# jmloveyj/ros_navigation

Measured on AMD Instinct MI355X. Metric: replan cycles/sec (HIMM+VFH++A*) on 4096x4096 grid, higher is better.
Workload: dtype int32; 1 GPU; full replan loop on 4096x4096 f32 grid (res 0.05 m); one step = one turn of the 20-stage A* pipeline = 20 passes of [100032-ray HIMM batch + fused compose -> 256 VFH+ poses -> 256 grid-A* queries (one launch)]; 30% rectangle obstacles (seed 2); 4 ray batches / pose sets / query sets in rotation; cycles_per_pass=256, rays_per_pass=100032, rotating_input_sets=4, astar_queries_checked=15360, astar_queries_answered=15360, astar_bucket_width=128000, astar_pipeline_depth=20, parallelism=query-sharded x1, full=False

## Files before the change

### ros_navigation_amd/csrc/astar.hip

```cpp
#include "engine.hpp"

#include <algorithm>
#include <cfloat>
#include <cmath>
#include <cstdlib>
#include <cstring>
#include <chrono>
#include <thread>
#include <vector>

using namespace rna;

namespace {

constexpr int COST_D = 1414;

struct HostTrace {
  bool on = getenv("RNA_HOST_TRACE") != nullptr;
  double us[8] = {};
  long n = 0, queries = 0;
  std::chrono::steady_clock::time_point t;
  void start() { if (on) t = std::chrono::steady_clock::now(); }
  void lap(int k) {
    if (!on) return;
// ... 65 lines not shown
          for (int c = skip; c < e->cu_count && c < 512; ++c) mask[c >> 5] |= 1u << (c & 31);
          RNA_HIP(e, hipExtStreamCreateWithCUMask(&a.side[d], (uint32_t)words, mask));
        } else {
          RNA_HIP(e, hipStreamCreateWithPriority(&a.side[d], hipStreamNonBlocking, prio_lo));
        }
      }
      RNA_HIP(e, hipEventCreateWithFlags(&a.done[d], hipEventDisableTiming));
      RNA_HIP(e, hipEventCreateWithFlags(&a.snap_done[d], hipEventDisableTiming));
    }
    a.snap_pending[d] = false;
    a.busy[d] = false;
    a.stage_seq[d] = 0;
  }
  if (a.depth > 1) {
    RNA_HIP(e, hipEventCreateWithFlags(&a.ev_init, hipEventDisableTiming));
    RNA_HIP(e, hipEventCreateWithFlags(&a.ev_prep, hipEventDisableTiming));
    a.ring_n = 2 * a.depth;
    a.ring_stride = tsa_ring_bytes(e, a.max_queries);
    if ((rc = dev_alloc(e, &a.ring_mem, a.ring_stride * (size_t)a.ring_n)) != RNA_OK) return rc;
    RNA_HIP(e, hipMemsetAsync(a.ring_mem, 0, a.ring_stride * (size_t)a.ring_n, e->stream));
    for (int r = 0; r < a.ring_n; ++r) {
      RNA_HIP(e, hipEventCreateWithFlags(&a.ring_free[r], hipEventDisableTiming));
      a.ring_used[r] = false;
    }
  }
  if (a.g_retry[0]) {
    RNA_HIP(e, hipHostMalloc(reinterpret_cast<void**>(&a.retry_flag), AstarDevice::MAX_DEPTH * sizeof(int), hipHostMallocCoherent));
    for (int d = 0; d < AstarDevice::MAX_DEPTH; ++d) a.retry_flag[d] = 0;
  }
  a.launches = 0;
  if ((rc = dev_alloc(e, &a.queries_dev, (size_t)a.max_queries)) != RNA_OK) { astar_release(e); return rc; }
  if ((rc = dev_alloc(e, &a.results_dev, (size_t)a.max_queries)) != RNA_OK) { astar_release(e); return rc; }
  return RNA_OK;
}

static int alloc_stages(rna_engine* e) {
  const int rc = alloc_stages_impl(e);
  if (rc != RNA_OK) {
    const std::string why = e->err;
    (void)astar_release(e);
    e->err = why;
  }
  return rc;
}
// ... 171 lines not shown
#ifdef RNA_TSA_STATS
  tsa_stats_dump();
#endif
  for (int d = 0; d < AstarDevice::MAX_DEPTH; ++d) {
    dev_free(&a.g[d]); dev_free(&a.rev[d]);
    if (a.tsa_aux[d]) { (void)hipFree(a.tsa_aux[d]); a.tsa_aux[d] = nullptr; }
    dev_free(&a.g_retry[d]);
    if (a.tsa_aux_retry[d]) { (void)hipFree(a.tsa_aux_retry[d]); a.tsa_aux_retry[d] = nullptr; }
    if (a.side[d]) { (void)hipStreamDestroy(a.side[d]); a.side[d] = nullptr; }
    if (a.done[d]) { (void)hipEventDestroy(a.done[d]); a.done[d] = nullptr; }
    if (a.snap_done[d]) { (void)hipEventDestroy(a.snap_done[d]); a.snap_done[d] = nullptr; }
    a.snap_pending[d] = false;
    a.busy[d] = false;
  }
  if (a.ev_init) { (void)hipEventDestroy(a.ev_init); a.ev_init = nullptr; }
  if (a.ev_prep) { (void)hipEventDestroy(a.ev_prep); a.ev_prep = nullptr; }
  for (int r = 0; r < AstarDevice::MAX_RING; ++r) {
    if (a.ring_free[r]) { (void)hipEventDestroy(a.ring_free[r]); a.ring_free[r] = nullptr; }
    a.ring_used[r] = false;
  }
  dev_free(&a.ring_mem);
  a.ring_n = 0;
  if (a.retry_flag) { (void)hipHostFree(a.retry_flag); a.retry_flag = nullptr; }
  for (int d = 0; d < AstarDevice::MAX_DEPTH; ++d) a.retry_armed[d] = false;
  dev_free(&a.queries_dev); dev_free(&a.results_dev); dev_free(&a.paths_dev);
  a.paths_cap = 0;
  a.last_queries = nullptr; a.last_results = nullptr; a.last_n = 0;
  return RNA_OK;
}
}

extern "C" int rna_astar_configure(rna_engine* e, int max_queries, int queue_capacity, int bucket_width) {
  if (!e || max_queries < 0 || queue_capacity < 0 || bucket_width < 0) return RNA_EINVAL;
  if (bucket_width != 0 && bucket_width < 2 * COST_D) return fail(e, RNA_EINVAL, "bucket_width must be >= 2828");
  RNA_ENTER(e);
  RNA_HIP(e, hipStreamSynchronize(e->stream));
  AstarDevice& a = e->astar;
// ... 145 lines not shown
```

### ros_navigation_amd/csrc/astar_tile.hip

```cpp
#include "engine.hpp"
#include <algorithm>
#include <cstring>
#include <vector>

using namespace rna;

namespace rna {

constexpr int TI = 64, TJ = 16;
constexpr int TILE_WORDS = TI * TJ;
constexpr int AUX_WORDS = 64;
constexpr int MASK_STRIDE = TILE_WORDS + 32 + 128;
constexpr int TSA_WAVES = 8;
constexpr int TSA_WAVES_PER_EU = 8;
constexpr int TSA_HPASS = 4;
constexpr int TSA_IDLE_SLEEP = 4;
constexpr int TSA_PRIO_FIRST = 0;
constexpr int TSA_BT_PRIO = 3;
constexpr int TSA_SCOPE = __HIP_MEMORY_SCOPE_AGENT;
constexpr int TSA_MAX_TILE_WORDS = 2048;
constexpr int COST_S = 1000, COST_D = 1414;
constexpr int INF = 0x7fffffff;
constexpr int KU = 0x40000000;
constexpr int SCR_CNT = 84 + 192 + 48 + 64;
// ... 78 lines not shown
  unsigned* paux;
  unsigned* tmap;
  unsigned* owner;
  int* nalloc;
  uint8_t* nbr_tm;
  int* perm;
  int* ticket;
  int cap;
};
__host__ __device__ inline size_t tsa_align256(size_t x) { return (x + 255) & ~(size_t)255; }
constexpr int TSA_COUNTER_WORDS = 16;
__host__ __device__ inline unsigned long long* tsa_counters_of(const TsaStage& S) {
  return reinterpret_cast<unsigned long long*>(reinterpret_cast<char*>(S.nalloc) - TSA_COUNTER_WORDS * sizeof(unsigned long long));
}

__global__ void __launch_bounds__(256) tsa_snapshot_kernel(const uint8_t* __restrict__ nbr, int rows, int cols, int tiles_i, int tiles_j,
                                                             uint8_t* __restrict__ nbr_tm, int s0, int s1) {
  __shared__ unsigned s_free[256];
  const int a = threadIdx.x & 63, bq = threadIdx.x >> 6;
  for (int t = blockIdx.x; t < tiles_i * tiles_j; t += gridDim.x) {
    const int i = (t % tiles_i) * TI + a, j0 = (t / tiles_i) * TJ + bq * 4;
    unsigned v = 0u;
    if (i < rows) {
      const int bi = i + s0 >= rows ? i + s0 - rows : i + s0;
#pragma unroll
      for (int k = 0; k < 4; ++k)
        if (j0 + k < cols) {
          const int bj = j0 + k + s1 >= cols ? j0 + k + s1 - cols : j0 + k + s1;
          v |= (unsigned)nbr[(size_t)bj * rows + bi] << (8 * k);
        }
    }
    uint8_t* out = nbr_tm + (size_t)t * MASK_STRIDE;
    reinterpret_cast<unsigned*>(out)[a * 4 + bq] = v;
    if (a == 0) reinterpret_cast<unsigned*>(out + TILE_WORDS)[bq] = v;
    if (a == TI - 1) reinterpret_cast<unsigned*>(out + TILE_WORDS + 16)[bq] = v;
    s_free[threadIdx.x] = (((v & 0xffu) != 0u) ? 1u : 0u) | (((v & 0xff00u) != 0u) ? 2u : 0u) | (((v & 0xff0000u) != 0u) ? 4u : 0u) |
                          (((v & 0xff000000u) != 0u) ? 8u : 0u);
    __syncthreads();
    if (bq == 0)
      reinterpret_cast<unsigned short*>(out + TILE_WORDS + 32)[a] =
          (unsigned short)(s_free[a] | (s_free[64 + a] << 4) | (s_free[128 + a] << 8) | (s_free[192 + a] << 12));
    __syncthreads();
  }
}
__global__ void __launch_bounds__(256) tsa_prepare_kernel(TsaStage S, const rna_astar_query* __restrict__ queries, int n, int rows, int cols,
                                                          int ranked, int* __restrict__ served) {
  extern __shared__ int s_key[];
  if (threadIdx.x == 0) *S.ticket = 0;
  if (served && threadIdx.x < TSA_RETRY) served[threadIdx.x] = -1;
  if (served && threadIdx.x == TSA_RETRY) served[TSA_RETRY] = 0;
  if (!ranked) {
    for (int i = threadIdx.x; i < n; i += blockDim.x) S.perm[i] = i;
    return;
  }
  const int ncell = rows * cols;
  for (int i = threadIdx.x; i < n; i += blockDim.x) {
    const rna_astar_query q = queries[i];
    int key = -1;
    if (q.start >= 0 && q.goal >= 0 && q.start < ncell && q.goal < ncell) {
      const int di = abs(q.start % rows - q.goal % rows), dj = abs(q.start / rows - q.goal / rows);
      key = di > dj ? di : dj;
    }
    s_key[i] = key;
  }
  __syncthreads();
  for (int i = threadIdx.x; i < n; i += blockDim.x) {
    const int ki = s_key[i];
    int rank = 0;
    for (int j = 0; j < n; ++j) {
      const int kj = s_key[j];
      rank += (kj > ki || (kj == ki && j < i)) ? 1 : 0;
    }
    S.perm[rank] = i;
  }
}
__global__ void tsa_fill_pages_kernel(uint4* __restrict__ p, size_t n4) {
  const size_t step = (size_t)gridDim.x * blockDim.x;
  for (size_t w = (size_t)blockIdx.x * blockDim.x + threadIdx.x; w < n4; w += step) p[w] = make_uint4(0u, 0u, 0u, 0u);
}

#ifdef RNA_TSA_STATS
__device__ unsigned long long g_tsa_stat[32];
#define TSA_T(var) const unsigned long long var = wall_clock64()
#define TSA_ACC(slot, t0, t1) tsa_acc[slot] += (unsigned long long)((t1) - (t0))
#define TSA_CNT(slot, v) tsa_acc[slot] += (unsigned long long)(v)
#define TSA_ACC_PARAM , unsigned long long* tsa_acc
#define TSA_ACC_ARG , tsa_acc
#else
// ... 1240 lines not shown
  return RNA_OK;
}
int tsa_stage_prepare(rna_engine* e, int slot) {
  const TsaStage S = tsa_stage_view(e, slot);
  const size_t pages = (size_t)e->astar.max_queries * ((size_t)S.cap + 1);
  hipLaunchKernelGGL(tsa_fill_pages_kernel, dim3(8192), dim3(256), 0, e->stream, reinterpret_cast<uint4*>(S.pages),
                     pages * (TILE_WORDS + AUX_WORDS) / 4);
  RNA_HIP(e, hipGetLastError());
  return RNA_OK;
}

size_t tsa_ring_bytes(const rna_engine* e, int max_queries) {
  return 256 + tsa_align256((size_t)max_queries * sizeof(int)) + tsa_align256((size_t)tsa_ntile(e) * MASK_STRIDE);
}
static_assert(sizeof(TsaLaunch) <= sizeof(AstarDevice::last_launch[0]), "AstarDevice::last_launch holds a TsaLaunch");

int tsa_retry_launch(rna_engine* e, int slot, hipStream_t search_stream, int count) {
  AstarDevice& a = e->astar;
  TsaLaunch A;
  memcpy(&A, a.last_launch[slot], sizeof(A));
  A.retry = 1;
  A.retry_count = nullptr;
  A.S2 = tsa_retry_view(e, slot, A.S);
  for (int base = 0; base < count; base += TSA_RETRY) {
    A.retry_base = base;
    const int wgs = std::min(TSA_RETRY, count - base);
    if (a.depth > 1) hipLaunchKernelGGL((tsa_search_kernel<TSA_WAVES, true>), dim3(wgs), dim3(TSA_WAVES * 64), a.last_lds[slot], search_stream, A);
    else hipLaunchKernelGGL((tsa_search_kernel<16, true>), dim3(wgs), dim3(16 * 64), a.last_lds[slot], search_stream, A);
    RNA_HIP(e, hipGetLastError());
  }
// ... 8 lines not shown
  TsaStage S = tsa_stage_view(e, slot);
  hipStream_t prep_stream = search_stream;
  int ring = -1;
  if (ev_init) {
    ring = (int)(a.launches % (unsigned long long)a.ring_n);
    char* base = a.ring_mem + (size_t)ring * a.ring_stride;
    S.ticket = reinterpret_cast<int*>(base);
    S.perm = reinterpret_cast<int*>(base + 256);
    S.nbr_tm = reinterpret_cast<uint8_t*>(base + 256 + tsa_align256((size_t)a.max_queries * sizeof(int)));
    { const int rc = side_stream(e, &prep_stream); if (rc != RNA_OK) return rc; }
    RNA_HIP(e, hipEventRecord(ev_init, init_stream));
    RNA_HIP(e, hipStreamWaitEvent(prep_stream, ev_init, 0));
    if (a.ring_used[ring]) RNA_HIP(e, hipStreamWaitEvent(prep_stream, a.ring_free[ring], 0));
  }
  {
    KernelTimer kt(e, RNA_K_ASTAR_INIT, prep_stream);
    hipLaunchKernelGGL(tsa_snapshot_kernel, dim3(std::min(ti * tj, 4096)), dim3(256), 0, prep_stream, e->nbr, rows, cols, ti, tj, S.nbr_tm,
                       e->geom.start[0], e->geom.start[1]);
    RNA_HIP(e, hipGetLastError());
  }
  if (ev_init) {
    RNA_HIP(e, hipEventRecord(a.snap_done[slot], prep_stream));
    a.snap_pending[slot] = true;
  }
  {
    KernelTimer kt(e, RNA_K_ASTAR_RESET, prep_stream);
    const int ranked = n <= 2048 ? 1 : 0;
    hipLaunchKernelGGL(tsa_prepare_kernel, dim3(1), dim3(256), ranked ? (size_t)n * sizeof(int) : 0, prep_stream, S, q_dev, n, rows, cols, ranked,
                       a.g_retry[slot] ? tsa_retry_served(e, slot) : nullptr);
    RNA_HIP(e, hipGetLastError());
  }
  if (ev_init) {
    RNA_HIP(e, hipEventRecord(a.ev_prep, prep_stream));
    RNA_HIP(e, hipStreamWaitEvent(search_stream, a.ev_prep, 0));
  }
  {
    KernelTimer kt(e, RNA_K_ASTAR_SEARCH, search_stream);
    const size_t nt_bytes = (size_t)((ti * tj + 31) / 32) * sizeof(unsigned);
    TsaLaunch A;
    memset(&A, 0, sizeof(A));
    A.rows = rows; A.cols = cols; A.tiles_i = ti; A.tiles_j = tj; A.s0 = e->geom.start[0]; A.s1 = e->geom.start[1];
    A.queries = q_dev; A.S = S; A.bucket_width = a.bucket_width; A.paths = paths_dev; A.max_path_len = max_len;
    A.rev_all = a.rev[slot]; A.rev_cap = a.rev_cap; A.results = res_dev;
    A.retry = 0; A.n = n; A.S2 = S;
    A.prio_first = a.depth > 1 ? TSA_PRIO_FIRST : 0;
    if (const char* pf = getenv("RNA_TSA_PRIO_FIRST")) A.prio_first = atoi(pf);
    size_t lds_dyn = 4 * nt_bytes;
    if (const char* pad = getenv("RNA_TSA_LDS_PAD")) lds_dyn += (size_t)atoi(pad);
    const bool can_retry = a.g_retry[slot] != nullptr && a.retry_flag != nullptr;
// ... 83 lines not shown
```

### ros_navigation_amd/csrc/compose_dev.hpp

```cpp
#pragma once
#include "engine.hpp"

namespace rna {

__device__ __forceinline__ bool cell_blocked(float v) { return !(v != v) && v > 0.0f; }

constexpr int COMPOSE_BLK_BYTES = (TILE + 2) * (TILE + 2);

__device__ __forceinline__ void compose_nbr_tile(uint8_t* __restrict__ blk, int tt, uint8_t* __restrict__ nbr, float* __restrict__ master,
                                                 const float* __restrict__ laser, const unsigned* __restrict__ dirty,
                                                 unsigned* __restrict__ next_dirty, int rows, int cols, int tiles_i, int tiles_j) {
  const int ti = tt % tiles_i, tj = tt / tiles_i;
  const unsigned char* dflag = reinterpret_cast<const unsigned char*>(dirty);
  unsigned dmask = 0u;
  for (int dj = -1; dj <= 1; ++dj)
    for (int di = -1; di <= 1; ++di) {
      const int a = ti + di, b = tj + dj;
      if (a < 0 || b < 0 || a >= tiles_i || b >= tiles_j) continue;
      if (dflag[b * tiles_i + a]) dmask |= 1u << ((dj + 1) * 3 + di + 1);
    }
  if (threadIdx.x == 0) reinterpret_cast<volatile unsigned char*>(next_dirty)[tj * tiles_i + ti] = 0;
  if (!dmask) return;
  const bool own = (dmask >> 4) & 1u;
  __syncthreads();
  const int i0 = ti * TILE - 1, j0 = tj * TILE - 1;
  for (int k = threadIdx.x; k < (TILE + 2) * (TILE + 2); k += blockDim.x) {
// ... 17 lines not shown
    if (i >= rows || j >= cols) continue;
    const uint8_t* c = &blk[(lj + 1) * (TILE + 2) + (li + 1)];
    constexpr int S = TILE + 2;
    unsigned m = 0;
    if (!c[0]) {
      const bool up = !c[-1], dn = !c[1], lf = !c[-S], rt = !c[S];
      if (lf && up && !c[-S - 1]) m |= 1u;
      if (lf) m |= 2u;
      if (lf && dn && !c[-S + 1]) m |= 4u;
      if (up) m |= 8u;
      if (dn) m |= 16u;
      if (rt && up && !c[S - 1]) m |= 32u;
      if (rt) m |= 64u;
      if (rt && dn && !c[S + 1]) m |= 128u;
    }
    nbr[(size_t)j * rows + i] = (uint8_t)m;
  }
}

}
```

### ros_navigation_amd/csrc/engine.hip

```cpp
#include "engine.hpp"
#include "compose_dev.hpp"

#include <cmath>
#include <dirent.h>
#include <unistd.h>
#include <cstdlib>
#include <cstring>
#include <limits>

using namespace rna;

__global__ void fill_f32_kernel(float* __restrict__ p, size_t n, float v) {
  size_t i = (size_t)blockIdx.x * blockDim.x + threadIdx.x;
  const size_t stride = (size_t)gridDim.x * blockDim.x;
  for (; i < n; i += stride) p[i] = v;
}

__global__ void compose_dirty_tiles_kernel(float* __restrict__ master, const float* __restrict__ laser,
                                           const unsigned* __restrict__ dirty, int rows, int cols, int tiles_i) {
  const int ti = blockIdx.x, tj = blockIdx.y;
  const int t = tj * tiles_i + ti;
  if (!reinterpret_cast<const unsigned char*>(dirty)[t]) return;
  const int i0 = ti * TILE, j0 = tj * TILE;
  const int li = threadIdx.x & (TILE - 1);
  for (int c = threadIdx.x >> 6; c < TILE; c += 4) {
    const int i = i0 + li, j = j0 + c;
    if (i < rows && j < cols) {
      const size_t lin = (size_t)j * rows + i;
      master[lin] = laser[lin];
    }
  }
}


__global__ void nbr_mask_tiles_kernel(uint8_t* __restrict__ nbr, const float* __restrict__ master,
                                      const unsigned* __restrict__ dirty, int all, int rows, int cols,
                                      int tiles_i, int tiles_j, int s0, int s1) {
  const int ti = blockIdx.x, tj = blockIdx.y;
  if (!all) {
    bool need = false;
    for (int dj = -1; dj <= 1 && !need; ++dj)
      for (int di = -1; di <= 1; ++di) {
        const int a = ti + di, b = tj + dj;
        if (a < 0 || b < 0 || a >= tiles_i || b >= tiles_j) continue;
        const int t = b * tiles_i + a;
        if (reinterpret_cast<const unsigned char*>(dirty)[t]) { need = true; break; }
      }
    if (!need) return;
  }
  __shared__ uint8_t blk[(TILE + 2) * (TILE + 2)];
  const int i0 = ti * TILE - 1, j0 = tj * TILE - 1;
  for (int k = threadIdx.x; k < (TILE + 2) * (TILE + 2); k += blockDim.x) {
// ... 18 lines not shown
    unsigned m = 0;
    if (!c[0]) {
      const bool up = !c[-1], dn = !c[1], lf = !c[-S], rt = !c[S];
      if (lf && up && !c[-S - 1]) m |= 1u;
      if (lf) m |= 2u;
      if (lf && dn && !c[-S + 1]) m |= 4u;
      if (up) m |= 8u;
      if (dn) m |= 16u;
      if (rt && up && !c[S - 1]) m |= 32u;
      if (rt) m |= 64u;
      if (rt && dn && !c[S + 1]) m |= 128u;
    }
    int bi = i + s0, bj = j + s1;
    if (bi >= rows) bi -= rows;
    if (bj >= cols) bj -= cols;
    nbr[(size_t)bj * rows + bi] = (uint8_t)m;
  }
}

__global__ void __launch_bounds__(256) compose_nbr_tiles_kernel(uint8_t* __restrict__ nbr, float* __restrict__ master, const float* __restrict__ laser,
                                                                const unsigned* __restrict__ dirty, unsigned* __restrict__ next_dirty, int rows,
                                                                int cols, int tiles_i, int tiles_j) {
  __shared__ uint8_t blk[(TILE + 2) * (TILE + 2)];
  for (int tt = blockIdx.x; tt < tiles_i * tiles_j; tt += gridDim.x)
    compose_nbr_tile(blk, tt, nbr, master, laser, dirty, next_dirty, rows, cols, tiles_i, tiles_j);
}

__global__ void clear_region_kernel(float* __restrict__ p, int rows, int i0, int ni, int j0, int nj) {
  const size_t n = (size_t)ni * nj;
  size_t k = (size_t)blockIdx.x * blockDim.x + threadIdx.x;
  const size_t stride = (size_t)gridDim.x * blockDim.x;
  const float nanv = __int_as_float(0x7fc00000);
  for (; k < n; k += stride) {
    const int i = i0 + (int)(k % ni), j = j0 + (int)(k / ni);
    p[(size_t)j * rows + i] = nanv;
  }
}

__global__ void __launch_bounds__(256) pack_tiles_kernel(const float* __restrict__ layer, int rows, int tiles_i,
                                                         const int32_t* __restrict__ tiles, int wi0, int wi1, int wj0,
// ... 115 lines not shown
      const int words = (prop.multiProcessorCount + 31) / 32 < 16 ? (prop.multiProcessorCount + 31) / 32 : 16;
      if (hipExtStreamCreateWithCUMask(&e->stream, (uint32_t)words, mask) != hipSuccess) return bail(RNA_EHIP);
    } else if (hipStreamCreateWithPriority(&e->stream, hipStreamNonBlocking, prio_hi) != hipSuccess) return bail(RNA_EHIP);
  }
  for (int l = 0; l < RNA_NUM_LAYERS; ++l) {
    if ((rc = dev_alloc(e, &e->layer[l], e->ncell)) != RNA_OK) return bail(rc);
    if ((rc = fill_layer(e, e->layer[l], std::numeric_limits<float>::quiet_NaN())) != RNA_OK) return bail(rc);
  }
  const size_t words = ((size_t)e->tiles_i * e->tiles_j + 3) / 4;
  if ((rc = dev_alloc(e, &e->dirty_tiles, words)) != RNA_OK) return bail(rc);
  if (hipMemsetAsync(e->dirty_tiles, 0, words * sizeof(unsigned), e->stream) != hipSuccess) return bail(RNA_EHIP);
  if ((rc = dev_alloc(e, &e->last_dirty, words)) != RNA_OK) return bail(rc);
  if (hipMemsetAsync(e->last_dirty, 0, words * sizeof(unsigned), e->stream) != hipSuccess) return bail(RNA_EHIP);
  if ((rc = dev_alloc(e, &e->nbr, e->ncell)) != RNA_OK) return bail(rc);
  e->nbr_all_dirty = true;
  if (hipStreamSynchronize(e->stream) != hipSuccess) return bail(RNA_EHIP);
  *out = e;
  return RNA_OK;
}

extern "C" void rna_destroy(rna_engine* e) {
  if (!e) return;
  (void)hipSetDevice(e->device);
  if (e->stream) (void)sync_all(e);
  himm_release(e);
  vfh_release(e);
  astar_release(e);
  footprint_release(e);
  goal_field_release(e);
  for (int l = 0; l < RNA_NUM_LAYERS; ++l) dev_free(&e->layer[l]);
  dev_free(&e->dirty_tiles);
  dev_free(&e->last_dirty);
  dev_free(&e->tile_list);
  dev_free(&e->nbr);
  (void)profile_flush(e);
  for (hipEvent_t ev : e->free_events) (void)hipEventDestroy(ev);
  e->free_events.clear();
  if (e->vfh_stream) (void)hipStreamDestroy(e->vfh_stream);
  if (e->ev_vfh_go) (void)hipEventDestroy(e->ev_vfh_go);
  if (e->ev_vfh_done) (void)hipEventDestroy(e->ev_vfh_done);
  if (e->stream) (void)hipStreamDestroy(e->stream);
  delete e;
}

extern "C" int rna_get_geometry(const rna_engine* e, rna_geometry* o) {
  if (!e || !o) return RNA_EINVAL;
  for (int a = 0; a < 2; ++a) {
    o->length[a] = e->geom.len[a];
    o->position[a] = e->geom.pos[a];
// ... 417 lines not shown
  int src = sync_all(e);
  if (src != RNA_OK) return src;
  for (auto& slot : e->prof) {
    for (auto& pr : slot.pending) {
      float ms = 0;
      if (hipEventElapsedTime(&ms, pr.first, pr.second) == hipSuccess) { slot.total_ms += ms; slot.launches += 1; }
      e->free_events.push_back(pr.first);
      e->free_events.push_back(pr.second);
    }
    slot.pending.clear();
  }
  e->pending_events = 0;
  return RNA_OK;
}

int map_prepare_nbr(rna_engine* e) {
  if (!e->nbr_all_dirty) return RNA_OK;
  { const int rc = side_join(e); if (rc != RNA_OK) return rc; }
  if (e->robot_r > 0.0) {
    const int rc = footprint_refresh(e, 1);
    if (rc != RNA_OK) return rc;
    e->nbr_all_dirty = false;
    return RNA_OK;
  }
  KernelTimer kt(e, RNA_K_NBRMASK);
  hipLaunchKernelGGL(nbr_mask_tiles_kernel, dim3(e->tiles_i, e->tiles_j), dim3(256), 0, e->stream, e->nbr,
                     e->layer[RNA_LAYER_MASTER], e->dirty_tiles, 1, e->geom.size[0], e->geom.size[1], e->tiles_i,
                     e->tiles_j, e->geom.start[0], e->geom.start[1]);
  RNA_HIP(e, hipGetLastError());
  e->nbr_all_dirty = false;
  return RNA_OK;
}

}

extern "C" int rna_compose_master(rna_engine* e, int mode) {
  if (!e || (mode != 0 && mode != 1)) return RNA_EINVAL;
  RNA_ENTER(e);
  e->map_epoch++;
  const size_t words = ((size_t)e->tiles_i * e->tiles_j + 3) / 4;
  const bool full = (mode == 1) || e->laser_all_dirty || e->master_diverged;
  const bool moved = e->geom.start[0] != 0 || e->geom.start[1] != 0;
  if (!full && !moved && !e->nbr_all_dirty && e->robot_r == 0.0) {
    KernelTimer kt(e, RNA_K_COMPOSE);
    static const int wgs_per_cu = [] { const char* v = getenv("RNA_COMPOSE_WGS_PER_CU"); const int n = v ? atoi(v) : 0; return n > 0 ? n : 16; }();
    hipLaunchKernelGGL(compose_nbr_tiles_kernel, dim3(std::min(e->tiles_i * e->tiles_j, wgs_per_cu * e->cu_count)), dim3(256), 0, e->stream, e->nbr,
                       e->layer[RNA_LAYER_MASTER], e->layer[RNA_LAYER_LASER], e->dirty_tiles, e->last_dirty, e->geom.size[0],
                       e->geom.size[1], e->tiles_i, e->tiles_j);
    RNA_HIP(e, hipGetLastError());
    std::swap(e->dirty_tiles, e->last_dirty);
    return RNA_OK;
  }
  {
    KernelTimer kt(e, RNA_K_COMPOSE);
    if (full) {
      RNA_HIP(e, hipMemcpyAsync(e->layer[RNA_LAYER_MASTER], e->layer[RNA_LAYER_LASER], e->ncell * sizeof(float),
                                hipMemcpyDeviceToDevice, e->stream));
    } else {
      hipLaunchKernelGGL(compose_dirty_tiles_kernel, dim3(e->tiles_i, e->tiles_j), dim3(256), 0, e->stream,
                         e->layer[RNA_LAYER_MASTER], e->layer[RNA_LAYER_LASER], e->dirty_tiles, e->geom.size[0],
                         e->geom.size[1], e->tiles_i);
      RNA_HIP(e, hipGetLastError());
    }
  }
  if (e->laser_all_dirty || e->master_diverged || moved) {
    e->nbr_all_dirty = true;
  } else if (!e->nbr_all_dirty && e->robot_r > 0.0) {
    const int rc = footprint_refresh(e, 0);
    if (rc != RNA_OK) return rc;
  } else if (!e->nbr_all_dirty) {
    KernelTimer kt(e, RNA_K_NBRMASK);
    hipLaunchKernelGGL(nbr_mask_tiles_kernel, dim3(e->tiles_i, e->tiles_j), dim3(256), 0, e->stream, e->nbr,
                       e->layer[RNA_LAYER_MASTER], e->dirty_tiles, 0, e->geom.size[0], e->geom.size[1], e->tiles_i,
                       e->tiles_j, 0, 0);
    RNA_HIP(e, hipGetLastError());
  }
  if (full) {
    RNA_HIP(e, hipMemsetAsync(e->last_dirty, 1, words * sizeof(unsigned), e->stream));
  } else {
    RNA_HIP(e, hipMemcpyAsync(e->last_dirty, e->dirty_tiles, words * sizeof(unsigned), hipMemcpyDeviceToDevice, e->stream));
  }
  RNA_HIP(e, hipMemsetAsync(e->dirty_tiles, 0, words * sizeof(unsigned), e->stream));
  e->laser_all_dirty = false;
  e->master_diverged = false;
  return RNA_OK;
}

extern "C" int rna_move(rna_engine* e, double nx, double ny, int* moved) {
  if (!e) return RNA_EINVAL;
// ... 78 lines not shown
```

### ros_navigation_amd/csrc/engine.hpp

```cpp
#pragma once

#include <hip/hip_runtime.h>

#include <cstdint>
#include <cstdio>
#include <string>
#include <vector>

#include "../../include/rna.h"
#include "gridmath.hpp"

namespace rna {

constexpr int TILE = 64;

struct HimmSlot { int cell; int head; int len; int offset; };

struct HimmScratch {
  int cap_rays = 0;
  int n_slots = 0;
  rna_ray* rays_dev = nullptr;
  int4* desc = nullptr;
  int* ncells = nullptr;
  int* next = nullptr;
  HimmSlot* slots = nullptr;
  int* seqs = nullptr;
  unsigned* before = nullptr;
  unsigned* after = nullptr;
  int* total = nullptr;
// ... 45 lines not shown
  int32_t* g_retry[MAX_DEPTH] = {};
  void* tsa_aux_retry[MAX_DEPTH] = {};
  hipStream_t side[MAX_DEPTH] = {};
  hipEvent_t done[MAX_DEPTH] = {};
  hipEvent_t snap_done[MAX_DEPTH] = {};
  bool snap_pending[MAX_DEPTH] = {};
  bool busy[MAX_DEPTH] = {};
  unsigned long long stage_seq[MAX_DEPTH] = {};
  hipEvent_t ev_init = nullptr;
  static constexpr int MAX_RING = 2 * MAX_DEPTH;
  int ring_n = 0;
  char* ring_mem = nullptr;
  size_t ring_stride = 0;
  hipEvent_t ring_free[MAX_RING] = {};
  bool ring_used[MAX_RING] = {};
  hipEvent_t ev_prep = nullptr;
  int* retry_flag = nullptr;
  bool retry_armed[MAX_DEPTH] = {};
  int last_retried[MAX_DEPTH] = {};
  size_t last_lds[MAX_DEPTH] = {};
  alignas(8) unsigned char last_launch[MAX_DEPTH][384] = {};
  unsigned long long launches = 0;
  int last_slot = 0;
  size_t field_stride = 0;
  rna_astar_query* queries_dev = nullptr;
  rna_astar_result* results_dev = nullptr;
  int32_t* paths_dev = nullptr;
  int paths_cap = 0;
  const rna_astar_query* last_queries = nullptr;
  const rna_astar_result* last_results = nullptr;
  int last_n = 0;
// ... 35 lines not shown
  hipStream_t stream = nullptr;
  hipStream_t vfh_stream = nullptr;
  hipEvent_t ev_vfh_go = nullptr, ev_vfh_done = nullptr;
  bool vfh_pending = false;
  size_t ncell = 0;
  float* layer[RNA_NUM_LAYERS] = {nullptr, nullptr, nullptr};
  int tiles_i = 0, tiles_j = 0;
  unsigned* dirty_tiles = nullptr;
  unsigned* last_dirty = nullptr;
  int32_t* tile_list = nullptr;
  int tile_list_cap = 0;
  bool laser_all_dirty = false;
  bool master_diverged = false;
  uint8_t* nbr = nullptr;
  bool nbr_all_dirty = true;
  double robot_r = 0.0;
  unsigned long long* fp_bits = nullptr;
  rna::FootprintPlan fp{};
  int2* fp_ties = nullptr;
  int fp_ties_cap = 0;
  unsigned long long map_epoch = 0;
  rna::GoalField gfield;
  rna::HimmScratch himm;
  rna::VfhDevice vfh;
  rna::AstarDevice astar;
  int profiling = 0;
  rna::ProfSlot prof[RNA_K_COUNT];
  std::vector<hipEvent_t> free_events;
  size_t pending_events = 0;
  std::string err;
// ... 21 lines not shown
  hipEvent_t a = nullptr, b = nullptr;
  static hipEvent_t take(rna_engine* e) {
    hipEvent_t ev = nullptr;
    if (!e->free_events.empty()) { ev = e->free_events.back(); e->free_events.pop_back(); }
    else if (hipEventCreate(&ev) != hipSuccess) ev = nullptr;
    return ev;
  }
  hipStream_t st;
  KernelTimer(rna_engine* eng, int kid, hipStream_t stream = nullptr) : e(eng), id(kid), st(stream ? stream : eng->stream) {
    if (!wanted()) return;
    if (e->pending_events > 16384) (void)profile_flush(e);
    a = take(e);
    b = take(e);
    if (a) (void)hipEventRecord(a, st);
  }
  bool wanted() const { return e->profiling == 1 || (e->profiling == 2 && (id == RNA_K_ASTAR_SEARCH || id == RNA_K_ASTAR_RESET)); }
  ~KernelTimer() {
    if (!wanted() || !a || !b) return;
    (void)hipEventRecord(b, st);
    e->prof[id].pending.emplace_back(a, b);
    e->pending_events += 2;
  }
};

template <typename T>
inline int dev_alloc(rna_engine* e, T** p, size_t n) {
  if (*p) { (void)hipFree(*p); *p = nullptr; }
  if (n == 0) return RNA_OK;
  hipError_t st = hipMalloc((void**)p, n * sizeof(T));
  if (st != hipSuccess) { *p = nullptr; return fail(e, RNA_ENOMEM, std::string("hipMalloc: ") + hipGetErrorString(st)); }
  return RNA_OK;
// ... 7 lines not shown
int side_join(rna_engine* e);
int side_stream(rna_engine* e, hipStream_t* out);
int astar_settle(rna_engine* e);
#define RNA_ENTER(e)                                        \
  do {                                                      \
    RNA_HIP(e, hipSetDevice((e)->device));                  \
    const int rc_join_ = rna::side_join(e);                 \
    if (rc_join_ != RNA_OK) return rc_join_;                \
  } while (0)
#define RNA_ENTER_NOJOIN(e) RNA_HIP(e, hipSetDevice((e)->device))

int himm_release(rna_engine* e);
int vfh_release(rna_engine* e);
int astar_release(rna_engine* e);
int map_prepare_nbr(rna_engine* e);
int footprint_refresh(rna_engine* e, int all);
int footprint_release(rna_engine* e);
int goal_field_release(rna_engine* e);
int sync_all(rna_engine* e);
bool tsa_supported(const rna_engine* e);
int tsa_tiles(const rna_engine* e);
size_t tsa_pool_bytes(int max_queries, int cap);
size_t tsa_aux_bytes(const rna_engine* e, int max_queries, int cap);
int tsa_stage_prepare(rna_engine* e, int slot);
constexpr int TSA_RETRY = 8;
size_t tsa_retry_pool_bytes(const rna_engine* e);
size_t tsa_retry_aux_bytes(const rna_engine* e);
int tsa_retry_prepare(rna_engine* e, int slot);
size_t tsa_ring_bytes(const rna_engine* e, int max_queries);
int tsa_retry_launch(rna_engine* e, int slot, hipStream_t search_stream, int count);
// ... 7 lines not shown
```

### ros_navigation_amd/csrc/footprint.hip

```cpp
#include "engine.hpp"
#include "compose_dev.hpp"

#include <algorithm>
#include <cmath>
#include <vector>

using namespace rna;

namespace {

constexpr int FP_MAX_R = 63;
constexpr int FP_ROWS = TILE + 2 * (FP_MAX_R + 1);
constexpr int FP_BLK = TILE + 2;

__device__ bool disc_blocked(const Geom& g, const float* __restrict__ master, double px, double py, double radius) {
  const double r2 = radius * radius;
  double tl[2] = {px + radius, py + radius}, br[2] = {px - radius, py - radius};
  limit_position_to_range(g, tl);
  limit_position_to_range(g, br);
  int s[2] = {0, 0}, t[2] = {0, 0};
  (void)index_from_position(g, tl[0], tl[1], s);
  (void)index_from_position(g, br[0], br[1], t);
  int su[2], tu[2];
  unwrap_index(g, s, su);
// ... 28 lines not shown
  unwrap_index(g, t, tu);
  const int lo0 = i - K < 0 ? 0 : i - K, hi0 = i + K > g.size[0] - 1 ? g.size[0] - 1 : i + K;
  const int lo1 = j - K < 0 ? 0 : j - K, hi1 = j + K > g.size[1] - 1 ? g.size[1] - 1 : j + K;
  return su[0] >= 0 && su[0] <= lo0 && tu[0] >= hi0 && tu[0] < g.size[0] && su[1] >= 0 && su[1] <= lo1 && tu[1] >= hi1 &&
         tu[1] < g.size[1];
}

__device__ __forceinline__ unsigned long long funnel64(unsigned long long lo, unsigned long long hi, int s) {
  return s ? (lo >> s) | (hi << (64 - s)) : lo;
}

}

__global__ void __launch_bounds__(256) footprint_tiles_kernel(uint8_t* __restrict__ nbr, unsigned long long* __restrict__ bits,
                                                              const float* __restrict__ master, const unsigned* __restrict__ dirty,
                                                              int all, Geom g, FootprintPlan P, const int2* __restrict__ ties) {
  const int ti = blockIdx.x, tj = blockIdx.y;
  const int tiles_i = gridDim.x, tiles_j = gridDim.y;
  const int rows = g.size[0], cols = g.size[1];
  if (!all) {
    bool need = false;
    for (int dj = -1; dj <= 1 && !need; ++dj)
      for (int di = -1; di <= 1; ++di) {
        const int a = ti + di, b = tj + dj;
        if (a < 0 || b < 0 || a >= tiles_i || b >= tiles_j) continue;
        if (reinterpret_cast<const unsigned char*>(dirty)[b * tiles_i + a]) { need = true; break; }
      }
    if (!need) return;
  }
  __shared__ unsigned long long occ[FP_ROWS][4];
  __shared__ uint8_t blk[FP_BLK * FP_BLK];
// ... 75 lines not shown
    constexpr int S = FP_BLK;
    unsigned m = 0;
    if (!c[0]) {
      const bool up = !c[-1], dn = !c[1], lf = !c[-S], rt = !c[S];
      if (lf && up && !c[-S - 1]) m |= 1u;
      if (lf) m |= 2u;
      if (lf && dn && !c[-S + 1]) m |= 4u;
      if (up) m |= 8u;
      if (dn) m |= 16u;
      if (rt && up && !c[S - 1]) m |= 32u;
      if (rt) m |= 64u;
      if (rt && dn && !c[S + 1]) m |= 128u;
    }
    const int bi = i + g.start[0] >= rows ? i + g.start[0] - rows : i + g.start[0];
    const int bj = j + g.start[1] >= cols ? j + g.start[1] - cols : j + g.start[1];
    nbr[(size_t)bj * rows + bi] = (uint8_t)m;
  }
}

__global__ void blocked_bytes_kernel(uint8_t* __restrict__ out, const unsigned long long* __restrict__ bits, const float* __restrict__ master,
                                     int rows, int cols, int tiles_i, int s0, int s1) {
  const size_t n = (size_t)rows * cols;
  for (size_t k = (size_t)blockIdx.x * blockDim.x + threadIdx.x; k < n; k += (size_t)gridDim.x * blockDim.x) {
    if (!bits) { out[k] = cell_blocked(master[k]) ? 1 : 0; continue; }
    const int bi = (int)(k % rows), bj = (int)(k / rows);
    const int i = bi - s0 < 0 ? bi - s0 + rows : bi - s0, j = bj - s1 < 0 ? bj - s1 + cols : bj - s1;
    const unsigned long long w = bits[((size_t)(j / TILE) * tiles_i + i / TILE) * TILE + (j % TILE)];
    out[k] = (uint8_t)((w >> (i % TILE)) & 1ull);
  }
}

// ... 40 lines not shown
}

}

namespace rna {

int footprint_release(rna_engine* e) {
  dev_free(&e->fp_bits);
  dev_free(&e->fp_ties);
  e->fp_ties_cap = 0;
  return RNA_OK;
}

int footprint_refresh(rna_engine* e, int all) {
  const Geom& g = e->geom;
  if (!e->fp_bits) {
    const int rc = dev_alloc(e, &e->fp_bits, (size_t)e->tiles_i * e->tiles_j * TILE);
    if (rc != RNA_OK) return rc;
    all = 1;
  }
  const double mag = geometry_magnitude(g, e->robot_r);
  if (e->fp.r != e->robot_r || e->fp.res != g.res || mag > e->fp.mag) {
    std::vector<int2> ties;
    const FootprintPlan P = make_plan(g, e->robot_r, 2.0 * mag, ties);
    RNA_HIP(e, hipStreamSynchronize(e->stream));
    if ((int)ties.size() > e->fp_ties_cap) {
      const int rc = dev_alloc(e, &e->fp_ties, ties.size());
      if (rc != RNA_OK) { e->fp_ties_cap = 0; return rc; }
      e->fp_ties_cap = (int)ties.size();
    }
    if (!ties.empty()) RNA_HIP(e, hipMemcpy(e->fp_ties, ties.data(), ties.size() * sizeof(int2), hipMemcpyHostToDevice));
    e->fp = P;
  }
  KernelTimer kt(e, RNA_K_FOOTPRINT);
  hipLaunchKernelGGL(footprint_tiles_kernel, dim3(e->tiles_i, e->tiles_j), dim3(256), 0, e->stream, e->nbr, e->fp_bits,
                     e->layer[RNA_LAYER_MASTER], e->dirty_tiles, all, g, e->fp, e->fp_ties);
  RNA_HIP(e, hipGetLastError());
  return RNA_OK;
}

}

extern "C" int rna_astar_set_robot_radius(rna_engine* e, double radius) {
  if (!e) return RNA_EINVAL;
  if (!(radius >= 0.0) || !(radius <= (double)FP_MAX_R * e->geom.res))
    return fail(e, RNA_EINVAL, "robot radius must satisfy 0 <= r and r / resolution <= 63");
  RNA_ENTER(e);
  e->robot_r = radius;
  e->map_epoch++;
  e->nbr_all_dirty = true;
  return RNA_OK;
// ... 63 lines not shown
```

Measured before the change: 164,100 replan cycles/s.

## Stamp changed nbr tiles and snapshot only changed tiles; fuse prepare into snapshot

Mask writers now write a neighbor byte only when it changes and stamp the containing search tile with a serial number. The A* snapshot kernel compares those stamps against a per-ring mark and re-copies only tiles changed since the last snapshot into that ring slot, falling back to a full copy when geometry or generation changes. The separate prepare kernel is folded into block 0 of the snapshot launch, removing one launch and one event wait. The cost is a read-before-write on every mask cell, extra stamp bookkeeping, and correctness depending on every writer maintaining the stamps.

```diff
diff --git a/ros_navigation_amd/csrc/astar.hip b/ros_navigation_amd/csrc/astar.hip
--- a/ros_navigation_amd/csrc/astar.hip
+++ b/ros_navigation_amd/csrc/astar.hip
@@ -103,7 +103,6 @@
   }
   if (a.depth > 1) {
     RNA_HIP(e, hipEventCreateWithFlags(&a.ev_init, hipEventDisableTiming));
-    RNA_HIP(e, hipEventCreateWithFlags(&a.ev_prep, hipEventDisableTiming));
     a.ring_n = 2 * a.depth;
     a.ring_stride = tsa_ring_bytes(e, a.max_queries);
     if ((rc = dev_alloc(e, &a.ring_mem, a.ring_stride * (size_t)a.ring_n)) != RNA_OK) return rc;
@@ -117,6 +116,7 @@
     RNA_HIP(e, hipHostMalloc(reinterpret_cast<void**>(&a.retry_flag), AstarDevice::MAX_DEPTH * sizeof(int), hipHostMallocCoherent));
     for (int d = 0; d < AstarDevice::MAX_DEPTH; ++d) a.retry_flag[d] = 0;
   }
+  for (AstarDevice::SnapMark& m : a.snap_mark) m.valid = false;
   a.launches = 0;
   if ((rc = dev_alloc(e, &a.queries_dev, (size_t)a.max_queries)) != RNA_OK) { astar_release(e); return rc; }
   if ((rc = dev_alloc(e, &a.results_dev, (size_t)a.max_queries)) != RNA_OK) { astar_release(e); return rc; }
@@ -318,13 +318,13 @@
     a.busy[d] = false;
   }
   if (a.ev_init) { (void)hipEventDestroy(a.ev_init); a.ev_init = nullptr; }
-  if (a.ev_prep) { (void)hipEventDestroy(a.ev_prep); a.ev_prep = nullptr; }
   for (int r = 0; r < AstarDevice::MAX_RING; ++r) {
     if (a.ring_free[r]) { (void)hipEventDestroy(a.ring_free[r]); a.ring_free[r] = nullptr; }
     a.ring_used[r] = false;
   }
   dev_free(&a.ring_mem);
   a.ring_n = 0;
+  for (AstarDevice::SnapMark& m : a.snap_mark) m.valid = false;
   if (a.retry_flag) { (void)hipHostFree(a.retry_flag); a.retry_flag = nullptr; }
   for (int d = 0; d < AstarDevice::MAX_DEPTH; ++d) a.retry_armed[d] = false;
   dev_free(&a.queries_dev); dev_free(&a.results_dev); dev_free(&a.paths_dev);
diff --git a/ros_navigation_amd/csrc/astar_tile.hip b/ros_navigation_amd/csrc/astar_tile.hip
--- a/ros_navigation_amd/csrc/astar_tile.hip
+++ b/ros_navigation_amd/csrc/astar_tile.hip
@@ -116,38 +116,34 @@
   return reinterpret_cast<unsigned long long*>(reinterpret_cast<char*>(S.nalloc) - TSA_COUNTER_WORDS * sizeof(unsigned long long));
 }
 
-__global__ void __launch_bounds__(256) tsa_snapshot_kernel(const uint8_t* __restrict__ nbr, int rows, int cols, int tiles_i, int tiles_j,
-                                                             uint8_t* __restrict__ nbr_tm, int s0, int s1) {
-  __shared__ unsigned s_free[256];
+__device__ __forceinline__ void tsa_snapshot_tile(int t, const uint8_t* __restrict__ nbr, int rows, int cols, int tiles_i,
+                                                  uint8_t* __restrict__ nbr_tm, int s0, int s1, unsigned* s_free) {
   const int a = threadIdx.x & 63, bq = threadIdx.x >> 6;
-  for (int t = blockIdx.x; t < tiles_i * tiles_j; t += gridDim.x) {
-    const int i = (t % tiles_i) * TI + a, j0 = (t / tiles_i) * TJ + bq * 4;
-    unsigned v = 0u;
-    if (i < rows) {
-      const int bi = i + s0 >= rows ? i + s0 - rows : i + s0;
+  const int i = (t % tiles_i) * TI + a, j0 = (t / tiles_i) * TJ + bq * 4;
+  unsigned v = 0u;
+  if (i < rows) {
+    const int bi = i + s0 >= rows ? i + s0 - rows : i + s0;
 #pragma unroll
-      for (int k = 0; k < 4; ++k)
-        if (j0 + k < cols) {
-          const int bj = j0 + k + s1 >= cols ? j0 + k + s1 - cols : j0 + k + s1;
-          v |= (unsigned)nbr[(size_t)bj * rows + bi] << (8 * k);
-        }
-    }
-    uint8_t* out = nbr_tm + (size_t)t * MASK_STRIDE;
-    reinterpret_cast<unsigned*>(out)[a * 4 + bq] = v;
-    if (a == 0) reinterpret_cast<unsigned*>(out + TILE_WORDS)[bq] = v;
-    if (a == TI - 1) reinterpret_cast<unsigned*>(out + TILE_WORDS + 16)[bq] = v;
-    s_free[threadIdx.x] = (((v & 0xffu) != 0u) ? 1u : 0u) | (((v & 0xff00u) != 0u) ? 2u : 0u) | (((v & 0xff0000u) != 0u) ? 4u : 0u) |
-                          (((v & 0xff000000u) != 0u) ? 8u : 0u);
-    __syncthreads();
-    if (bq == 0)
-      reinterpret_cast<unsigned short*>(out + TILE_WORDS + 32)[a] =
-          (unsigned short)(s_free[a] | (s_free[64 + a] << 4) | (s_free[128 + a] << 8) | (s_free[192 + a] << 12));
-    __syncthreads();
-  }
-}
-__global__ void __launch_bounds__(256) tsa_prepare_kernel(TsaStage S, const rna_astar_query* __restrict__ queries, int n, int rows, int cols,
-                                                          int ranked, int* __restrict__ served) {
-  extern __shared__ int s_key[];
+    for (int k = 0; k < 4; ++k)
+      if (j0 + k < cols) {
+        const int bj = j0 + k + s1 >= cols ? j0 + k + s1 - cols : j0 + k + s1;
+        v |= (unsigned)nbr[(size_t)bj * rows + bi] << (8 * k);
+      }
+  }
+  uint8_t* out = nbr_tm + (size_t)t * MASK_STRIDE;
+  reinterpret_cast<unsigned*>(out)[a * 4 + bq] = v;
+  if (a == 0) reinterpret_cast<unsigned*>(out + TILE_WORDS)[bq] = v;
+  if (a == TI - 1) reinterpret_cast<unsigned*>(out + TILE_WORDS + 16)[bq] = v;
+  s_free[threadIdx.x] = (((v & 0xffu) != 0u) ? 1u : 0u) | (((v & 0xff00u) != 0u) ? 2u : 0u) | (((v & 0xff0000u) != 0u) ? 4u : 0u) |
+                        (((v & 0xff000000u) != 0u) ? 8u : 0u);
+  __syncthreads();
+  if (bq == 0)
+    reinterpret_cast<unsigned short*>(out + TILE_WORDS + 32)[a] =
+        (unsigned short)(s_free[a] | (s_free[64 + a] << 4) | (s_free[128 + a] << 8) | (s_free[192 + a] << 12));
+  __syncthreads();
+}
+__device__ __forceinline__ void tsa_prepare(const TsaStage& S, const rna_astar_query* __restrict__ queries, int n, int rows, int cols, int ranked,
+                                            int* __restrict__ served, int* s_key) {
   if (threadIdx.x == 0) *S.ticket = 0;
   if (served && threadIdx.x < TSA_RETRY) served[threadIdx.x] = -1;
   if (served && threadIdx.x == TSA_RETRY) served[TSA_RETRY] = 0;
@@ -174,6 +170,34 @@
       rank += (kj > ki || (kj == ki && j < i)) ? 1 : 0;
     }
     S.perm[rank] = i;
+  }
+}
+__global__ void __launch_bounds__(256) tsa_snapshot_kernel(const uint8_t* __restrict__ nbr, int rows, int cols, int tiles_i, int tiles_j,
+                                                             uint8_t* __restrict__ nbr_tm, int s0, int s1, const unsigned* __restrict__ stamp,
+                                                             unsigned since, int full, TsaStage S, const rna_astar_query* __restrict__ queries,
+                                                             int n, int ranked, int* __restrict__ served) {
+  extern __shared__ int s_key[];
+  __shared__ unsigned s_free[256];
+  __shared__ int s_list[256];
+  __shared__ int s_n;
+  if (blockIdx.x == 0) {
+    tsa_prepare(S, queries, n, rows, cols, ranked, served, s_key);
+    return;
+  }
+  const int b = blockIdx.x - 1, G = gridDim.x - 1, ntile = tiles_i * tiles_j;
+  if (full) {
+    for (int t = b; t < ntile; t += G) tsa_snapshot_tile(t, nbr, rows, cols, tiles_i, nbr_tm, s0, s1, s_free);
+    return;
+  }
+  for (int base = 0; base < ntile; base += 256 * G) {
+    if (threadIdx.x == 0) s_n = 0;
+    __syncthreads();
+    const int t = base + (int)threadIdx.x * G + b;
+    if (t < ntile && stamp[t] > since) s_list[atomicAdd(&s_n, 1)] = t;
+    __syncthreads();
+    const int cnt = s_n;
+    for (int k = 0; k < cnt; ++k) tsa_snapshot_tile(s_list[k], nbr, rows, cols, tiles_i, nbr_tm, s0, s1, s_free);
+    __syncthreads();
   }
 }
 __global__ void tsa_fill_pages_kernel(uint4* __restrict__ p, size_t n4) {
@@ -1444,6 +1468,7 @@
   return 256 + tsa_align256((size_t)max_queries * sizeof(int)) + tsa_align256((size_t)tsa_ntile(e) * MASK_STRIDE);
 }
 static_assert(sizeof(TsaLaunch) <= sizeof(AstarDevice::last_launch[0]), "AstarDevice::last_launch holds a TsaLaunch");
+static_assert(TI == TILE && TJ == STAMP_TJ, "rna_engine::nbr_stamp is kept per search tile by the mask writers (compose_dev.hpp, engine.hip, footprint.hip)");
 
 int tsa_retry_launch(rna_engine* e, int slot, hipStream_t search_stream, int count) {
   AstarDevice& a = e->astar;
@@ -1482,25 +1507,25 @@
     if (a.ring_used[ring]) RNA_HIP(e, hipStreamWaitEvent(prep_stream, a.ring_free[ring], 0));
   }
   {
+    AstarDevice::SnapMark& M = a.snap_mark[ring >= 0 ? ring : AstarDevice::MAX_RING + slot];
+    const int s0 = e->geom.start[0], s1 = e->geom.start[1];
+    bool full = !M.valid || M.gen != e->nbr_stamp_gen || M.rows != rows || M.cols != cols || M.s0 != s0 || M.s1 != s1 ||
+                e->nbr_full_serial > M.serial;
+    if (getenv("RNA_TSA_SNAPSHOT_FULL")) full = true;
+    const int ntile = ti * tj;
+    const int wgs = full ? std::min(ntile, 4096) : std::min((ntile + 15) / 16, 256);
+    const int ranked = n <= 2048 ? 1 : 0;
     KernelTimer kt(e, RNA_K_ASTAR_INIT, prep_stream);
-    hipLaunchKernelGGL(tsa_snapshot_kernel, dim3(std::min(ti * tj, 4096)), dim3(256), 0, prep_stream, e->nbr, rows, cols, ti, tj, S.nbr_tm,
-                       e->geom.start[0], e->geom.start[1]);
+    hipLaunchKernelGGL(tsa_snapshot_kernel, dim3(1 + wgs), dim3(256), ranked ? (size_t)n * sizeof(int) : 0, prep_stream, e->nbr, rows, cols, ti, tj,
+                       S.nbr_tm, s0, s1, e->nbr_stamp, M.serial, full ? 1 : 0, S, q_dev, n, ranked,
+                       a.g_retry[slot] ? tsa_retry_served(e, slot) : nullptr);
     RNA_HIP(e, hipGetLastError());
+    M = AstarDevice::SnapMark{true, e->nbr_serial, e->nbr_stamp_gen, rows, cols, s0, s1};
   }
   if (ev_init) {
     RNA_HIP(e, hipEventRecord(a.snap_done[slot], prep_stream));
     a.snap_pending[slot] = true;
-  }
-  {
-    KernelTimer kt(e, RNA_K_ASTAR_RESET, prep_stream);
-    const int ranked = n <= 2048 ? 1 : 0;
-    hipLaunchKernelGGL(tsa_prepare_kernel, dim3(1), dim3(256), ranked ? (size_t)n * sizeof(int) : 0, prep_stream, S, q_dev, n, rows, cols, ranked,
-                       a.g_retry[slot] ? tsa_retry_served(e, slot) : nullptr);
-    RNA_HIP(e, hipGetLastError());
-  }
-  if (ev_init) {
-    RNA_HIP(e, hipEventRecord(a.ev_prep, prep_stream));
-    RNA_HIP(e, hipStreamWaitEvent(search_stream, a.ev_prep, 0));
+    RNA_HIP(e, hipStreamWaitEvent(search_stream, a.snap_done[slot], 0));
   }
   {
     KernelTimer kt(e, RNA_K_ASTAR_SEARCH, search_stream);
diff --git a/ros_navigation_amd/csrc/compose_dev.hpp b/ros_navigation_amd/csrc/compose_dev.hpp
--- a/ros_navigation_amd/csrc/compose_dev.hpp
+++ b/ros_navigation_amd/csrc/compose_dev.hpp
@@ -9,7 +9,8 @@
 
 __device__ __forceinline__ void compose_nbr_tile(uint8_t* __restrict__ blk, int tt, uint8_t* __restrict__ nbr, float* __restrict__ master,
                                                  const float* __restrict__ laser, const unsigned* __restrict__ dirty,
-                                                 unsigned* __restrict__ next_dirty, int rows, int cols, int tiles_i, int tiles_j) {
+                                                 unsigned* __restrict__ next_dirty, int rows, int cols, int tiles_i, int tiles_j,
+                                                 unsigned* __restrict__ stamp, unsigned serial) {
   const int ti = tt % tiles_i, tj = tt / tiles_i;
   const unsigned char* dflag = reinterpret_cast<const unsigned char*>(dirty);
   unsigned dmask = 0u;
@@ -57,7 +58,11 @@
       if (rt) m |= 64u;
       if (rt && dn && !c[S + 1]) m |= 128u;
     }
-    nbr[(size_t)j * rows + i] = (uint8_t)m;
+    const size_t lin = (size_t)j * rows + i;
+    if (nbr[lin] != (uint8_t)m) {
+      nbr[lin] = (uint8_t)m;
+      stamp[(size_t)(j / STAMP_TJ) * tiles_i + ti] = serial;
+    }
   }
 }
 
diff --git a/ros_navigation_amd/csrc/engine.hip b/ros_navigation_amd/csrc/engine.hip
--- a/ros_navigation_amd/csrc/engine.hip
+++ b/ros_navigation_amd/csrc/engine.hip
@@ -35,7 +35,7 @@
 
 __global__ void nbr_mask_tiles_kernel(uint8_t* __restrict__ nbr, const float* __restrict__ master,
                                       const unsigned* __restrict__ dirty, int all, int rows, int cols,
-                                      int tiles_i, int tiles_j, int s0, int s1) {
+                                      int tiles_i, int tiles_j, int s0, int s1, unsigned* __restrict__ stamp, unsigned serial) {
   const int ti = blockIdx.x, tj = blockIdx.y;
   if (!all) {
     bool need = false;
@@ -84,16 +84,22 @@
     int bi = i + s0, bj = j + s1;
     if (bi >= rows) bi -= rows;
     if (bj >= cols) bj -= cols;
-    nbr[(size_t)bj * rows + bi] = (uint8_t)m;
+    const size_t lin = (size_t)bj * rows + bi;
+    if (!stamp) {
+      nbr[lin] = (uint8_t)m;
+    } else if (nbr[lin] != (uint8_t)m) {
+      nbr[lin] = (uint8_t)m;
+      stamp[(size_t)(j / STAMP_TJ) * tiles_i + ti] = serial;
+    }
   }
 }
 
 __global__ void __launch_bounds__(256) compose_nbr_tiles_kernel(uint8_t* __restrict__ nbr, float* __restrict__ master, const float* __restrict__ laser,
                                                                 const unsigned* __restrict__ dirty, unsigned* __restrict__ next_dirty, int rows,
-                                                                int cols, int tiles_i, int tiles_j) {
+                                                                int cols, int tiles_i, int tiles_j, unsigned* __restrict__ stamp, unsigned serial) {
   __shared__ uint8_t blk[(TILE + 2) * (TILE + 2)];
   for (int tt = blockIdx.x; tt < tiles_i * tiles_j; tt += gridDim.x)
-    compose_nbr_tile(blk, tt, nbr, master, laser, dirty, next_dirty, rows, cols, tiles_i, tiles_j);
+    compose_nbr_tile(blk, tt, nbr, master, laser, dirty, next_dirty, rows, cols, tiles_i, tiles_j, stamp, serial);
 }
 
 __global__ void clear_region_kernel(float* __restrict__ p, int rows, int i0, int ni, int j0, int nj) {
@@ -239,6 +245,9 @@
   if (hipMemsetAsync(e->last_dirty, 0, words * sizeof(unsigned), e->stream) != hipSuccess) return bail(RNA_EHIP);
   if ((rc = dev_alloc(e, &e->nbr, e->ncell)) != RNA_OK) return bail(rc);
   e->nbr_all_dirty = true;
+  const size_t stamps = (size_t)e->tiles_i * ((e->geom.size[1] + STAMP_TJ - 1) / STAMP_TJ);
+  if ((rc = dev_alloc(e, &e->nbr_stamp, stamps)) != RNA_OK) return bail(rc);
+  if (hipMemsetAsync(e->nbr_stamp, 0, stamps * sizeof(unsigned), e->stream) != hipSuccess) return bail(RNA_EHIP);
   if (hipStreamSynchronize(e->stream) != hipSuccess) return bail(RNA_EHIP);
   *out = e;
   return RNA_OK;
@@ -258,6 +267,7 @@
   dev_free(&e->last_dirty);
   dev_free(&e->tile_list);
   dev_free(&e->nbr);
+  dev_free(&e->nbr_stamp);
   (void)profile_flush(e);
   for (hipEvent_t ev : e->free_events) (void)hipEventDestroy(ev);
   e->free_events.clear();
@@ -705,9 +715,23 @@
   return RNA_OK;
 }
 
+int nbr_next_serial(rna_engine* e, bool whole_layer, unsigned* serial) {
+  if (e->nbr_serial == 0xffffffffu) {
+    const size_t stamps = (size_t)e->tiles_i * ((e->geom.size[1] + STAMP_TJ - 1) / STAMP_TJ);
+    RNA_HIP(e, hipMemsetAsync(e->nbr_stamp, 0, stamps * sizeof(unsigned), e->stream));
+    e->nbr_serial = e->nbr_full_serial = 0;
+    e->nbr_stamp_gen += 1;
+  }
+  e->nbr_serial += 1;
+  if (whole_layer) e->nbr_full_serial = e->nbr_serial;
+  if (serial) *serial = e->nbr_serial;
+  return RNA_OK;
+}
+
 int map_prepare_nbr(rna_engine* e) {
   if (!e->nbr_all_dirty) return RNA_OK;
   { const int rc = side_join(e); if (rc != RNA_OK) return rc; }
+  { const int rc = nbr_next_serial(e, true, nullptr); if (rc != RNA_OK) return rc; }
   if (e->robot_r > 0.0) {
     const int rc = footprint_refresh(e, 1);
     if (rc != RNA_OK) return rc;
@@ -717,7 +741,7 @@
   KernelTimer kt(e, RNA_K_NBRMASK);
   hipLaunchKernelGGL(nbr_mask_tiles_kernel, dim3(e->tiles_i, e->tiles_j), dim3(256), 0, e->stream, e->nbr,
                      e->layer[RNA_LAYER_MASTER], e->dirty_tiles, 1, e->geom.size[0], e->geom.size[1], e->tiles_i,
-                     e->tiles_j, e->geom.start[0], e->geom.start[1]);
+                     e->tiles_j, e->geom.start[0], e->geom.start[1], nullptr, 0u);
   RNA_HIP(e, hipGetLastError());
   e->nbr_all_dirty = false;
   return RNA_OK;
@@ -733,11 +757,13 @@
   const bool full = (mode == 1) || e->laser_all_dirty || e->master_diverged;
   const bool moved = e->geom.start[0] != 0 || e->geom.start[1] != 0;
   if (!full && !moved && !e->nbr_all_dirty && e->robot_r == 0.0) {
+    unsigned serial = 0;
+    { const int rc = nbr_next_serial(e, false, &serial); if (rc != RNA_OK) return rc; }
     KernelTimer kt(e, RNA_K_COMPOSE);
     static const int wgs_per_cu = [] { const char* v = getenv("RNA_COMPOSE_WGS_PER_CU"); const int n = v ? atoi(v) : 0; return n > 0 ? n : 16; }();
     hipLaunchKernelGGL(compose_nbr_tiles_kernel, dim3(std::min(e->tiles_i * e->tiles_j, wgs_per_cu * e->cu_count)), dim3(256), 0, e->stream, e->nbr,
                        e->layer[RNA_LAYER_MASTER], e->layer[RNA_LAYER_LASER], e->dirty_tiles, e->last_dirty, e->geom.size[0],
-                       e->geom.size[1], e->tiles_i, e->tiles_j);
+                       e->geom.size[1], e->tiles_i, e->tiles_j, e->nbr_stamp, serial);
     RNA_HIP(e, hipGetLastError());
     std::swap(e->dirty_tiles, e->last_dirty);
     return RNA_OK;
@@ -760,10 +786,12 @@
     const int rc = footprint_refresh(e, 0);
     if (rc != RNA_OK) return rc;
   } else if (!e->nbr_all_dirty) {
+    unsigned serial = 0;
+    { const int rc = nbr_next_serial(e, false, &serial); if (rc != RNA_OK) return rc; }
     KernelTimer kt(e, RNA_K_NBRMASK);
     hipLaunchKernelGGL(nbr_mask_tiles_kernel, dim3(e->tiles_i, e->tiles_j), dim3(256), 0, e->stream, e->nbr,
                        e->layer[RNA_LAYER_MASTER], e->dirty_tiles, 0, e->geom.size[0], e->geom.size[1], e->tiles_i,
-                       e->tiles_j, 0, 0);
+                       e->tiles_j, 0, 0, e->nbr_stamp, serial);
     RNA_HIP(e, hipGetLastError());
   }
   if (full) {
diff --git a/ros_navigation_amd/csrc/engine.hpp b/ros_navigation_amd/csrc/engine.hpp
--- a/ros_navigation_amd/csrc/engine.hpp
+++ b/ros_navigation_amd/csrc/engine.hpp
@@ -13,6 +13,7 @@
 namespace rna {
 
 constexpr int TILE = 64;
+constexpr int STAMP_TJ = 16;
 
 struct HimmSlot { int cell; int head; int len; int offset; };
 
@@ -88,7 +89,8 @@
   size_t ring_stride = 0;
   hipEvent_t ring_free[MAX_RING] = {};
   bool ring_used[MAX_RING] = {};
-  hipEvent_t ev_prep = nullptr;
+  struct SnapMark { bool valid; unsigned serial, gen; int rows, cols, s0, s1; };
+  SnapMark snap_mark[MAX_RING + MAX_DEPTH] = {};
   int* retry_flag = nullptr;
   bool retry_armed[MAX_DEPTH] = {};
   int last_retried[MAX_DEPTH] = {};
@@ -154,6 +156,8 @@
   bool master_diverged = false;
   uint8_t* nbr = nullptr;
   bool nbr_all_dirty = true;
+  unsigned* nbr_stamp = nullptr;
+  unsigned nbr_serial = 0, nbr_full_serial = 0, nbr_stamp_gen = 0;
   double robot_r = 0.0;
   unsigned long long* fp_bits = nullptr;
   rna::FootprintPlan fp{};
@@ -205,7 +209,7 @@
     b = take(e);
     if (a) (void)hipEventRecord(a, st);
   }
-  bool wanted() const { return e->profiling == 1 || (e->profiling == 2 && (id == RNA_K_ASTAR_SEARCH || id == RNA_K_ASTAR_RESET)); }
+  bool wanted() const { return e->profiling == 1 || (e->profiling == 2 && (id == RNA_K_ASTAR_SEARCH || id == RNA_K_ASTAR_INIT)); }
   ~KernelTimer() {
     if (!wanted() || !a || !b) return;
     (void)hipEventRecord(b, st);
@@ -243,6 +247,7 @@
 int vfh_release(rna_engine* e);
 int astar_release(rna_engine* e);
 int map_prepare_nbr(rna_engine* e);
+int nbr_next_serial(rna_engine* e, bool whole_layer, unsigned* serial);
 int footprint_refresh(rna_engine* e, int all);
 int footprint_release(rna_engine* e);
 int goal_field_release(rna_engine* e);
diff --git a/ros_navigation_amd/csrc/footprint.hip b/ros_navigation_amd/csrc/footprint.hip
--- a/ros_navigation_amd/csrc/footprint.hip
+++ b/ros_navigation_amd/csrc/footprint.hip
@@ -66,7 +66,8 @@
 
 __global__ void __launch_bounds__(256) footprint_tiles_kernel(uint8_t* __restrict__ nbr, unsigned long long* __restrict__ bits,
                                                               const float* __restrict__ master, const unsigned* __restrict__ dirty,
-                                                              int all, Geom g, FootprintPlan P, const int2* __restrict__ ties) {
+                                                              int all, Geom g, FootprintPlan P, const int2* __restrict__ ties,
+                                                              unsigned* __restrict__ stamp, unsigned serial) {
   const int ti = blockIdx.x, tj = blockIdx.y;
   const int tiles_i = gridDim.x, tiles_j = gridDim.y;
   const int rows = g.size[0], cols = g.size[1];
@@ -172,7 +173,13 @@
     }
     const int bi = i + g.start[0] >= rows ? i + g.start[0] - rows : i + g.start[0];
     const int bj = j + g.start[1] >= cols ? j + g.start[1] - cols : j + g.start[1];
-    nbr[(size_t)bj * rows + bi] = (uint8_t)m;
+    const size_t lin = (size_t)bj * rows + bi;
+    if (!stamp) {
+      nbr[lin] = (uint8_t)m;
+    } else if (nbr[lin] != (uint8_t)m) {
+      nbr[lin] = (uint8_t)m;
+      stamp[(size_t)(j / STAMP_TJ) * tiles_i + ti] = serial;
+    }
   }
 }
 
@@ -243,6 +250,7 @@
 
 int footprint_refresh(rna_engine* e, int all) {
   const Geom& g = e->geom;
+  const bool whole_counted = all != 0;
   if (!e->fp_bits) {
     const int rc = dev_alloc(e, &e->fp_bits, (size_t)e->tiles_i * e->tiles_j * TILE);
     if (rc != RNA_OK) return rc;
@@ -261,9 +269,11 @@
     if (!ties.empty()) RNA_HIP(e, hipMemcpy(e->fp_ties, ties.data(), ties.size() * sizeof(int2), hipMemcpyHostToDevice));
     e->fp = P;
   }
+  unsigned serial = 0;
+  if (!all || !whole_counted) { const int rc = nbr_next_serial(e, all != 0, &serial); if (rc != RNA_OK) return rc; }
   KernelTimer kt(e, RNA_K_FOOTPRINT);
   hipLaunchKernelGGL(footprint_tiles_kernel, dim3(e->tiles_i, e->tiles_j), dim3(256), 0, e->stream, e->nbr, e->fp_bits,
-                     e->layer[RNA_LAYER_MASTER], e->dirty_tiles, all, g, e->fp, e->fp_ties);
+                     e->layer[RNA_LAYER_MASTER], e->dirty_tiles, all, g, e->fp, e->fp_ties, all ? nullptr : e->nbr_stamp, serial);
   RNA_HIP(e, hipGetLastError());
   return RNA_OK;
 }
```

Result: no change. 165,100 replan cycles/s, median of 6 (+0.6%).
